# TaceoLabs/collaborative-circom

Measured on AMD Instinct MI355X. Metric: Groth16 constraints/sec (BN254, 2^22 R1CS), one REP3 party's prove, higher is better.
Workload: dtype u32; 1 GPU; synthetic R1CS 2^22 constraints-domain BN254, REP3 co-groth16 (configs[2]); num_constraints=4194302, domain_size=4194304, nnz=12582906, msm=8 G1 + 2 G2 of ~2^22 points, ntt=12

## Files before the change

collaborative-circom_amd/csrc/capi_internal.hpp:

```cpp
#pragma once
#include "common.hpp"
#include "curve.hpp"
#include "subgroup.hpp"
#include "host_ec64.hpp"
#include "ntt_kernels.hpp"
#include "plonk_kernels.hpp"

#include <cmath>
#include <chrono>
#include <map>
#include <set>
#include <mutex>
#include <vector>

using namespace cg;

namespace cg {
struct MsmSortPtrs { const uint32_t* sorted; const uint32_t* offsets; const uint32_t* counts; uint32_t cap; const uint32_t* overflow; };
template <class Fr> int msm_sort_launch(hipStream_t st, const Fr* d_scalars, size_t n, int c, int nwin, int shared, char* scratch, MsmSortPtrs* out, hipEvent_t* evs);
template <class Fr> int msm_sort_direct_launch(hipStream_t st, const Fr* d_scalars, size_t n, int c, int nwin, int shared, uint32_t cap, char* scratch, MsmSortPtrs* out, hipEvent_t* evs);
inline size_t msm_sort_direct_scratch_bytes(size_t n, int c, int nwin, int shared, uint32_t cap) {
    const size_t nbuckets = (size_t)(shared ? 1 : nwin) << (c - 1);
    return align_up(nbuckets * cap * 4) + 2 * align_up(nbuckets * 4) + align_up(((nbuckets + 2047) / 2048) * 4) + 256;
}
template <class F> int msm_accumulate_batch(hipStream_t st, const MsmAccSet* sets, int nsets, size_t n, int c, int nwin, bool shared, uint32_t cap, hipEvent_t* evs, uint32_t chunk_request, bool g2_slices);
template <class F> int msm_reduce_batch(hipStream_t st2, const MsmRedSet* sets, int nsets, size_t n, int c, int nwin, bool shared, uint32_t cap, hipEvent_t* ev_merged, int n_merged,
                                        hipEvent_t* evs, uint32_t chunk_request);
template <class F> size_t msm_acc_scratch_bytes(size_t n, int c, int nwin, bool shared, uint32_t chunk_request);
template <class F> int precompute_window_launch(hipStream_t st, const Affine<F>* d_src, Affine<F>* d_dst, size_t n, int c);
template <class F> int check_on_curve_launch(hipStream_t st, const Affine<F>* d_pts, size_t n, const F& b, unsigned long long* d_counters);
template <class F, class Fr> int check_subgroup_launch(hipStream_t st, const Affine<F>* d_pts, size_t n, unsigned long long* d_counters);
template <class F> int check_subgroup_fast_launch(hipStream_t st, const Affine<F>* d_pts, size_t n, const FastSubgroup<F>& c, unsigned long long* d_counters);
inline size_t msm_sort_scratch_bytes(size_t n, int c, int nwin) {
    const size_t nbuckets = (size_t)nwin << (c - 1);
    const size_t entries = (size_t)nwin * n;
    return 2 * align_up(entries * 4) + 3 * align_up(nbuckets * 4) + align_up(((nbuckets + 2047) / 2048) * 4) + align_up(entries * 8) + 2 * align_up(4096 * 4) + 256;
}
template <class F> int pack_bases_launch(hipStream_t st, const uint8_t* d_raw, size_t n, size_t stride, long inf_off, Affine<F>* d_dst);
template <class F> int gather_points_launch(hipStream_t st, Affine<F>* d_dst, const Affine<F>* d_src, const uint32_t* d_idx, size_t n);
template <class Fr> int launch_vec_gather_idx(hipStream_t st, Fr* out, const Fr* in, const uint32_t* idx, size_t n, uint32_t base);
template <class F> int synth_points_launch(hipStream_t st, const XYZZ<F>* d_lo, const XYZZ<F>* d_hi, int log_t, size_t n, Affine<F>* d_out);
template <class F, class Fr> int fixed_base_mul_launch(hipStream_t st, const Affine<F>& g, const Fr* d_scalars, size_t n, Affine<F>* d_tab, Affine<F>* d_out);
template <class Fr> int launch_vec_binary(hipStream_t st, int op, Fr* out, const Fr* a, const Fr* b, size_t n);
int chacha12_fr_rand_launch(hipStream_t st, const uint32_t* key8, const uint32_t* mod8, int modulus_bits, uint64_t word_pos, uint64_t n_pairs, uint64_t n,
                            void* d_cand, uint32_t* d_tiles, unsigned long long* d_result, void* d_out);
template <class Fr> int launch_rep3_mul_local(hipStream_t st, Fr* out, const Fr* aa, const Fr* ab, const Fr* ba, const Fr* bb, const Fr* mask, size_t n);
template <class Fr> int launch_distribute_powers(hipStream_t st, Fr* v, size_t n, const Fr* lo, const Fr* hi, int log_lo);
template <class Fr> int launch_vec_count_noncanonical(hipStream_t st, const Fr* v, size_t n, unsigned long long* n_bad);
template <class Fr> int launch_vec_fill(hipStream_t st, Fr* v, size_t n, const Fr& value);
template <class Fr> int launch_vec_affine(hipStream_t st, Fr* out, const Fr* a, size_t n, const Fr& c, const Fr& d);
template <class Fr> int launch_vec_gather_strided(hipStream_t st, Fr* out, const Fr* in, size_t n, size_t offset, size_t stride);
template <class Fr> int launch_vec_lincomb(hipStream_t st, Fr* out, long long out_off, long long out_stride, size_t n, const LincombArgs<Fr>& a);
template <class Fr> int launch_shamir_share(hipStream_t st, const Fr* secrets, const Fr* coeffs, long long coeff_off, long long coeff_stride, size_t n, int degree,
                                            const ShareOuts<Fr>& o, long long out_off, long long out_stride);
template <class Fr> int launch_plonk_r2_factors(hipStream_t st, const PlonkR2Args<Fr>& g, size_t n);
template <class Fr> int launch_prefix_scan(hipStream_t st, int op, Fr* out, const Fr* in, size_t n, Fr* scratch);
template <class Fr> int launch_vec_inverse(hipStream_t st, Fr* out, const Fr* in, size_t n);
template <class Fr> int launch_plonk_additions(hipStream_t st, const uint32_t* order, size_t n, const uint32_t* ids, const Fr* coeffs, const Fr* pub, uint32_t n_inputs, int pc,
                                               Fr* ext_a, Fr* ext_b, size_t n_priv);
// ... 220 lines not shown
```

collaborative-circom_amd/csrc/fr_impl.hpp:

```cpp
#pragma once
#include "common.hpp"
#include "ntt_kernels.hpp"
#include "vec_kernels.hpp"
#include "plonk_kernels.hpp"
#include "msm_sort_kernels.hpp"

namespace cg {

template <class Fr> int launch_vec_binary(hipStream_t st, int op, Fr* out, const Fr* a, const Fr* b, size_t n) {
    if (!n) return 0;
    if (op == 0) hipLaunchKernelGGL((k_vec_binary<Fr, 0>), dim3(grid_for(n)), dim3(256), 0, st, out, a, b, n);
    else if (op == 1) hipLaunchKernelGGL((k_vec_binary<Fr, 1>), dim3(grid_for(n)), dim3(256), 0, st, out, a, b, n);
    else hipLaunchKernelGGL((k_vec_binary<Fr, 2>), dim3(grid_for(n)), dim3(256), 0, st, out, a, b, n);
    HIPCHK(hipGetLastError());
    return 0;
}
template <class Fr> int launch_rep3_mul_local(hipStream_t st, Fr* out, const Fr* aa, const Fr* ab, const Fr* ba, const Fr* bb, const Fr* mask, size_t n) {
    if (!n) return 0;
    hipLaunchKernelGGL((k_rep3_mul_local<Fr>), dim3(grid_for(n)), dim3(256), 0, st, out, aa, ab, ba, bb, mask, n);
    HIPCHK(hipGetLastError());
    return 0;
}
template <class Fr> int launch_vec_count_noncanonical(hipStream_t st, const Fr* v, size_t n, unsigned long long* n_bad) {
    if (!n) return 0;
// ... 157 lines not shown
        hipLaunchKernelGGL((k_bitrev_finish_lazy_small<Fr>), dim3(grid_for(n), nvec), dim3(256), 0, st, dst, src, log_m, scale, c_lo, c_hi, log_lo);
    HIPCHK(hipGetLastError());
    return 0;
}
template <class Fr> int launch_bitrev_scale(hipStream_t st, NttVecs dst, NttVecs src, int nvec, size_t n, int log_m, const Fr* scale, const Fr* c_lo, const Fr* c_hi, int log_lo) {
    if (log_m >= 2 * BITREV_B)
        hipLaunchKernelGGL((k_bitrev_scale<Fr>), dim3((unsigned)(n >> (2 * BITREV_B)), nvec), dim3(256), 0, st, dst, src, log_m, scale, c_lo, c_hi, log_lo);
    else
        hipLaunchKernelGGL((k_bitrev_scale_small<Fr>), dim3(grid_for(n), nvec), dim3(256), 0, st, dst, src, log_m, scale, c_lo, c_hi, log_lo);
    HIPCHK(hipGetLastError());
    return 0;
}

struct MsmSortPtrs { const uint32_t* sorted; const uint32_t* offsets; const uint32_t* counts; uint32_t cap; const uint32_t* overflow; };
inline bool msm_sort_use_partition(size_t n, int c, int nwin, int shared) {
    const size_t nbuckets = (size_t)(shared ? 1 : nwin) << (c - 1);
    const size_t nregions = (nbuckets + ((size_t)1 << PART_REGION_LOG) - 1) >> PART_REGION_LOG;
    return (size_t)nwin * n >= ((size_t)1 << 21) && nregions >= 8 && nregions <= PART_MAX_REGIONS;
}
inline size_t msm_sort_scratch_bytes(size_t n, int c, int nwin) {
    const size_t nbuckets = (size_t)nwin << (c - 1);
    const size_t entries = (size_t)nwin * n, ntiles = (entries + PART_TILE - 1) / PART_TILE;
    return 2 * align_up(entries * 4) + 3 * align_up(nbuckets * 4) + align_up(((nbuckets + SCAN_TILE - 1) / SCAN_TILE) * 4) +
           align_up(entries * 8) + 2 * align_up(PART_MAX_REGIONS * 4) + 256;
}
template <class Fr> int msm_sort_launch(hipStream_t st, const Fr* d_scalars, size_t n, int c, int nwin, int shared, char* scratch, MsmSortPtrs* out, hipEvent_t* evs) {
    const size_t nbuckets = (size_t)(shared ? 1 : nwin) << (c - 1);
    size_t off = 0;
    auto take = [&](size_t bytes) { void* p = scratch + off; off += align_up(bytes); return p; };
    int32_t* digits = (int32_t*)take((size_t)nwin * n * 4);
    uint32_t* sorted = (uint32_t*)take((size_t)nwin * n * 4);
    uint32_t* counts = (uint32_t*)take(nbuckets * 4);
    uint32_t* cursors = (uint32_t*)take(nbuckets * 4);
    uint32_t* offsets = (uint32_t*)take(nbuckets * 4);
    const size_t ntiles = (nbuckets + SCAN_TILE - 1) / SCAN_TILE;
    uint32_t* tile_sums = (uint32_t*)take(ntiles * 4);
    if (evs) HIPCHK(hipEventRecord(evs[0], st));
    const bool no_small = !global_option(CG_GOPT_SORT_SMALL);
    static PerDeviceOnce attr_small; static std::atomic<bool> small_unavailable{false};
    if (shared && !no_small && !small_unavailable.load(std::memory_order_relaxed) && attr_small.pending()) {
        if (hipFuncSetAttribute((const void*)k_msm_sort_small<Fr>, hipFuncAttributeMaxDynamicSharedMemorySize, (int)((2 * SORT_SMALL_MAX_BUCKETS + 1024) * 4)) == hipSuccess) attr_small.mark();
        else { (void)hipGetLastError(); small_unavailable.store(true); }
    }
    if (shared && !no_small && !small_unavailable.load(std::memory_order_relaxed) && nbuckets <= SORT_SMALL_MAX_BUCKETS && (size_t)nwin * n <= SORT_SMALL_MAX_ENTRIES && n <= (1u << 24)) {
        const size_t lds = (2 * nbuckets + 1024) * 4;
        hipLaunchKernelGGL((k_msm_sort_small<Fr>), dim3(1), dim3(1024), lds, st, d_scalars, (uint32_t)n, c, nwin, counts, offsets, sorted);
        if (evs) HIPCHK(hipEventRecord(evs[1], st));
        HIPCHK(hipGetLastError());
        out->sorted = sorted; out->offsets = offsets; out->counts = counts; out->cap = 0; out->overflow = nullptr;
        return 0;
    }
    HIPCHK(hipMemsetAsync(counts, 0, align_up(nbuckets * 4) * 2, st));
    if (msm_sort_use_partition(n, c, nwin, shared)) {
        const size_t entries = (size_t)nwin * n, ptiles = (entries + PART_TILE - 1) / PART_TILE;
        const uint32_t nregions = (uint32_t)((nbuckets + ((size_t)1 << PART_REGION_LOG) - 1) >> PART_REGION_LOG);
        uint64_t* items = (uint64_t*)take(entries * 8);
        uint32_t* region_total = (uint32_t*)take(PART_MAX_REGIONS * 4);
        uint32_t* region_cursor = (uint32_t*)take(PART_MAX_REGIONS * 4);
        uint32_t* total_items = (uint32_t*)take(4);
        const unsigned itiles = (unsigned)(((entries + ITEM_TILE - 1) / ITEM_TILE + 7) / 8 * 8);
        HIPCHK(hipMemsetAsync(region_total, 0, nregions * 4, st));
        hipLaunchKernelGGL((k_msm_digits_only<Fr>), dim3(grid_for(n)), dim3(256), 0, st, d_scalars, n, c, nwin, digits);
        hipLaunchKernelGGL(k_part_hist, dim3((unsigned)ptiles), dim3(256), nregions * 4, st, digits, n, c, nwin, shared, nregions, region_total);
        hipLaunchKernelGGL(k_part_region_scan, dim3(1), dim3(1024), 0, st, region_total, nregions, region_cursor, total_items);
        const bool staged = global_option(CG_GOPT_SORT_STAGING) != 0;
        if (staged && nregions <= STAGE_MAX_REGIONS) {
            static PerDeviceOnce attr_set;
            if (attr_set.pending()) {
                HIPCHK(hipFuncSetAttribute((const void*)k_part_scatter_staged, hipFuncAttributeMaxDynamicSharedMemorySize, (int)part_staged_lds(STAGE_MAX_REGIONS)));
                HIPCHK(hipFuncSetAttribute((const void*)k_items_scatter_staged, hipFuncAttributeMaxDynamicSharedMemorySize, (int)ITEMS_STAGED_LDS));
                attr_set.mark();
            }
            hipLaunchKernelGGL(k_part_scatter_staged, dim3((unsigned)ptiles), dim3(STAGE_THREADS), part_staged_lds(nregions), st, digits, n, c, nwin, shared, nregions, region_cursor, items);
        } else
        hipLaunchKernelGGL(k_part_scatter, dim3((unsigned)ptiles), dim3(256), nregions * 4, st, digits, n, c, nwin, shared, nregions, region_cursor, items);
        hipLaunchKernelGGL(k_items_hist, dim3(itiles), dim3(256), 0, st, items, total_items, counts);
        hipLaunchKernelGGL(k_scan_tile_sums, dim3((unsigned)ntiles), dim3(256), 0, st, counts, tile_sums, nbuckets, 0xffffffffu);
        hipLaunchKernelGGL(k_scan_exclusive, dim3(1), dim3(1024), 0, st, tile_sums, tile_sums, ntiles);
        hipLaunchKernelGGL(k_scan_tiles, dim3((unsigned)ntiles), dim3(256), 0, st, counts, tile_sums, offsets, nbuckets, 0xffffffffu);
        if (staged && nregions <= STAGE_MAX_REGIONS) hipLaunchKernelGGL(k_items_scatter_staged, dim3(itiles), dim3(STAGE_THREADS), ITEMS_STAGED_LDS, st, items, total_items, offsets, cursors, sorted);
        else hipLaunchKernelGGL(k_items_scatter, dim3(itiles), dim3(256), 0, st, items, total_items, offsets, cursors, sorted);
        if (evs) HIPCHK(hipEventRecord(evs[1], st));
        HIPCHK(hipGetLastError());
        out->sorted = sorted; out->offsets = offsets; out->counts = counts; out->cap = 0; out->overflow = nullptr;
        return 0;
    }
    hipLaunchKernelGGL((k_msm_digits<Fr>), dim3(grid_for(n)), dim3(256), 0, st, d_scalars, n, c, nwin, shared, digits, counts);
    hipLaunchKernelGGL(k_scan_tile_sums, dim3((unsigned)ntiles), dim3(256), 0, st, counts, tile_sums, nbuckets, 0xffffffffu);
    hipLaunchKernelGGL(k_scan_exclusive, dim3(1), dim3(1024), 0, st, tile_sums, tile_sums, ntiles);
    hipLaunchKernelGGL(k_scan_tiles, dim3((unsigned)ntiles), dim3(256), 0, st, counts, tile_sums, offsets, nbuckets, 0xffffffffu);
    hipLaunchKernelGGL(k_msm_scatter, dim3(grid_for((size_t)nwin * n)), dim3(256), 0, st, digits, n, c, nwin, shared, offsets, cursors, sorted);
    if (evs) HIPCHK(hipEventRecord(evs[1], st));
    HIPCHK(hipGetLastError());
    out->sorted = sorted; out->offsets = offsets; out->counts = counts; out->cap = 0; out->overflow = nullptr;
    return 0;
}
inline size_t msm_sort_direct_scratch_bytes(size_t n, int c, int nwin, int shared, uint32_t cap) {
    const size_t nbuckets = (size_t)(shared ? 1 : nwin) << (c - 1);
    return align_up(nbuckets * cap * 4) + 2 * align_up(nbuckets * 4) + align_up(((nbuckets + SCAN_TILE - 1) / SCAN_TILE) * 4) + 256;
}
template <class Fr> int msm_sort_direct_launch(hipStream_t st, const Fr* d_scalars, size_t n, int c, int nwin, int shared, uint32_t cap, char* scratch, MsmSortPtrs* out, hipEvent_t* evs) {
    const size_t nbuckets = (size_t)(shared ? 1 : nwin) << (c - 1);
// ... 58 lines not shown
```

collaborative-circom_amd/csrc/msm_impl.hpp:

```cpp
#pragma once
#include <cstdlib>
#include "common.hpp"
#include "msm_kernels.hpp"

namespace cg {

template <class B> constexpr int bitsum_items() { return BITSUM_ITEMS; }
inline int bitsum_items_for(uint32_t nb) { return nb <= 1024u ? 1 : BITSUM_ITEMS; }
template <class B> uint32_t bitsum_groups(uint32_t nb) { const uint32_t it = (uint32_t)bitsum_items_for(nb); return std::max<uint32_t>(1, (nb / 2 + 256 * it - 1) / (256 * it)); }

template <class F> struct IsFp2 { static constexpr bool value = false; };
template <class B> struct IsFp2<Fp2<B>> { static constexpr bool value = true; };
template <class F> constexpr size_t acc_resident_lanes() { return IsFp2<F>::value ? 0 : (size_t)256 * (sizeof(F) == 32 ? 3 : 2) * 256; }

template <class F>
size_t msm_acc_scratch_bytes(size_t n, int c, int nwin, bool shared, uint32_t chunk_request) {
    typedef typename BucketOf<F>::type B;
    MsmGeom g = msm_geom(n, c, nwin, shared, acc_resident_lanes<F>(), chunk_request, IsFp2<F>::value);
    g.bit_groups = bitsum_groups<B>(g.nb);
    return align_up(g.nbuckets * sizeof(B)) + align_up((size_t)g.nchunks * sizeof(B)) + align_up((size_t)g.nchunks * 4) +
           align_up(std::max({(size_t)g.nsets * g.segs, (size_t)64 * g.bit_groups, g.grid_partials()}) * sizeof(B)) + align_up((size_t)std::max(g.ngroups, 64) * sizeof(XYZZ<F>));
}

template <class F>
// ... 9 lines not shown
        partials = (B*)take(std::max({(size_t)g.nsets * g.segs, (size_t)64 * g.bit_groups, g.grid_partials()}) * sizeof(B));
        wsums = (XYZZ<F>*)take((size_t)std::max(g.ngroups, 64) * sizeof(XYZZ<F>));
    }
};
template <class F>
MsmGeom msm_geom_of(size_t n, int c, int nwin, bool shared, uint32_t chunk_request) {
    MsmGeom g = msm_geom(n, c, nwin, shared, acc_resident_lanes<F>(), chunk_request, IsFp2<F>::value);
    g.bit_groups = bitsum_groups<typename BucketOf<F>::type>(g.nb);
    return g;
}

template <class F>
int msm_accumulate_batch(hipStream_t st, const MsmAccSet* sets, int nsets, size_t n, int c, int nwin, bool shared, uint32_t cap, hipEvent_t* evs, uint32_t chunk_request, bool g2_slices) {
    if (nsets < 1 || nsets > ACC_MAX_SETS) return fail(CG_ERR_ARG, "internal: accumulation batch size");
    const MsmGeom g = msm_geom_of<F>(n, c, nwin, shared, chunk_request);
    typedef typename BucketOf<F>::type B;
    AccSets<F> S{};
    for (int i = 0; i < nsets; i++) {
        const AccScratch<F> sc(sets[i].scratch, g);
        S.bases[i] = (const Affine<F>*)sets[i].bases; S.sorted[i] = sets[i].sorted; S.offsets[i] = sets[i].offsets; S.counts[i] = sets[i].counts;
        S.buckets[i] = sc.buckets; S.cont[i] = sc.cont; S.cont_bucket[i] = sc.cont_bucket;
        S.table_stride[i] = (uint32_t)sets[i].table_stride; S.may_have_inf[i] = sets[i].may_have_inf ? 1u : 0u;
    }
    const ptrdiff_t stride = nsets > 1 ? sets[1].scratch - sets[0].scratch : 0;
    bool one_fill = stride > 0 && (size_t)(nsets - 1) * (size_t)stride + g.nbuckets * sizeof(B) <= ((size_t)8 << 20);
    for (int i = 2; i < nsets && one_fill; i++) one_fill = sets[i].scratch - sets[i - 1].scratch == stride;
    if (one_fill) HIPCHK(hipMemsetAsync(S.buckets[0], 0, (size_t)(nsets - 1) * (size_t)stride + g.nbuckets * sizeof(B), st));
    else for (int i = 0; i < nsets; i++) HIPCHK(hipMemsetAsync(S.buckets[i], 0, g.nbuckets * sizeof(B), st));
    if (evs) HIPCHK(hipEventRecord(evs[0], st));
    auto launch_acc = [&](auto kern, int T, size_t lds) -> int {
        if (lds > 0) { if (int rc = ensure_dynamic_lds((const void*)kern, lds)) return rc; }
        for (int i = 0; i < nsets; i++)
            hipLaunchKernelGGL(kern, dim3((g.nchunks + T - 1) / T), dim3(T), lds, st, S.bases[i], S.sorted[i], S.offsets[i], S.counts[i],
                               (uint32_t)g.nbuckets, g.chunk_len, g.nchunks, S.table_stride[i], cap, S.buckets[i], S.cont[i], S.cont_bucket[i], S.may_have_inf[i]);
        return 0;
    };
    int rc_acc;
    const char* var_s = tune_env("CG_ACC_VARIANT");
    const int variant = var_s ? atoi(var_s) : 3;
    auto launch_pf = [&](auto kern, int T, size_t lds) -> int {
        if (lds > 0) { if (int rc = ensure_dynamic_lds((const void*)kern, lds)) return rc; }
        const uint32_t groups = (g.nchunks + T - 1) / T;
        const uint32_t slice = lds > 0 && g2_slices ? 256u * (uint32_t)std::max<size_t>(1, ((size_t)160 << 10) / lds) : groups;
        for (uint32_t first = 0; first < groups; first += slice)
            hipLaunchKernelGGL(kern, dim3(std::min(slice, groups - first), (unsigned)nsets), dim3(T), lds, st, S, (uint32_t)g.nbuckets, g.chunk_len, g.nchunks, first * (uint32_t)T);
        return 0;
    };
    constexpr bool g2 = IsFp2<F>::value;
    constexpr int MINW1 = sizeof(F) == 32 ? 3 : 2;
    const size_t lds2 = g2 ? (size_t)128 * 4 * sizeof(typename LazyOf<F>::type) : 0;
    if (variant && cap == 0) {
// ... 172 lines not shown
```

collaborative-circom_amd/csrc/msm_kernels.hpp:

```cpp
#pragma once
#include <type_traits>
#include "common.hpp"
#include "subgroup.hpp"
#include "curve.hpp"
#include "lazy29.hpp"
#include "vec_kernels.hpp"
#include "msm_sort_kernels.hpp"

namespace cg {

template <class A>
__device__ __forceinline__ A ld_struct(const A* p) {
    static_assert(sizeof(A) % 16 == 0, "");
    A r;
    const uint4* q = reinterpret_cast<const uint4*>(p);
    uint4* d = reinterpret_cast<uint4*>(&r);
    _Pragma("unroll") for (int i = 0; i < (int)(sizeof(A) / 16); i++) d[i] = q[i];
    return r;
}
template <class A>
__device__ __forceinline__ void st_struct(A* p, const A& r) {
    uint4* q = reinterpret_cast<uint4*>(p);
    const uint4* d = reinterpret_cast<const uint4*>(&r);
    _Pragma("unroll") for (int i = 0; i < (int)(sizeof(A) / 16); i++) q[i] = d[i];
// ... 466 lines not shown
        const bool neg = (e0 >> 31) != 0;
        pos++;
        if constexpr (PF != 3) { e0 = e1; e1 = e2; }
        if (may_have_inf && p.is_inf()) continue;
        acc_madd(acc, p.x, p.y, neg);
    }
    if (continuation) acc_store<F>(acc, cont + q); else acc_store<F>(acc, buckets + b);
}

constexpr uint32_t MERGE_DIRECT_MAX = 12;
template <class B>
struct RedSets {
    B* buckets[RED_MAX_SETS]; B* cont[RED_MAX_SETS]; uint32_t* cont_bucket[RED_MAX_SETS];
    const uint32_t* offsets[RED_MAX_SETS]; const uint32_t* counts[RED_MAX_SETS];
    B* partials[RED_MAX_SETS]; void* wsums[RED_MAX_SETS];
};
template <class B>
__global__ void __launch_bounds__(64) k_msm_merge_direct(const RedSets<B> S, uint32_t nbuckets, uint32_t chunk_len, uint32_t nchunks, uint32_t cap) {
    B* __restrict__ buckets = S.buckets[blockIdx.y]; const B* __restrict__ cont = S.cont[blockIdx.y]; uint32_t* __restrict__ cont_bucket = S.cont_bucket[blockIdx.y];
    const uint32_t* __restrict__ offsets = S.offsets[blockIdx.y]; const uint32_t* __restrict__ counts = S.counts[blockIdx.y];
    const uint32_t b = blockIdx.x * blockDim.x + threadIdx.x;
    if (b >= nbuckets) return;
    const uint32_t cnt = cap ? min(counts[b], cap) : counts[b];
    if (cnt == 0) return;
    const uint32_t first = offsets[b], last = first + cnt - 1;
    const uint32_t q0 = first / chunk_len + 1, q1 = last / chunk_len;
    if (q0 > q1 || q1 - q0 >= MERGE_DIRECT_MAX || q1 >= nchunks) return;
    B acc = ld_struct(buckets + b);
    for (uint32_t q = q0; q <= q1; q++) { acc = bk_add_inl(acc, ld_struct(cont + q)); cont_bucket[q] = 0xffffffffu; }
    st_struct(buckets + b, acc);
}
constexpr uint32_t MERGE_GROUP = 64;
template <class B>
__global__ void __launch_bounds__(64) k_msm_merge_cont_l1(const RedSets<B> S, uint32_t nchunks) {
    B* __restrict__ cont = S.cont[blockIdx.y]; const uint32_t* __restrict__ cont_bucket = S.cont_bucket[blockIdx.y];
    const uint32_t q = blockIdx.x * blockDim.x + threadIdx.x;
    if (q >= nchunks) return;
    const uint32_t b = cont_bucket[q];
    if (b == 0xffffffffu) return;
    const bool run_start = q == 0 || cont_bucket[q - 1] != b;
    if (!run_start && (q % MERGE_GROUP) != 0) return;
    const uint32_t next_head = (q / MERGE_GROUP + 1) * MERGE_GROUP;
    if (q + 1 >= nchunks || q + 1 >= next_head || cont_bucket[q + 1] != b) return;
    B acc = ld_struct(cont + q);
    for (uint32_t r = q + 1; r < nchunks && r < next_head && cont_bucket[r] == b; r++) acc = bk_add_inl(acc, ld_struct(cont + r));
    st_struct(cont + q, acc);
}
// ... 296 lines not shown
```

collaborative-circom_amd/csrc/msm_sort_kernels.hpp:

```cpp
#pragma once
#include "field.hpp"
#include "vec_kernels.hpp"

namespace cg {

template <class Fr>
__global__ void __launch_bounds__(256) k_msm_digits(const Fr* __restrict__ scalars, size_t n, int c, int nwin, int shared,
                                                    int32_t* __restrict__ digits, uint32_t* __restrict__ counts) {
    const uint32_t nb = 1u << (c - 1);
    const uint32_t mask = (1u << c) - 1;
    for (size_t i = (size_t)blockIdx.x * blockDim.x + threadIdx.x; i < n; i += (size_t)gridDim.x * blockDim.x) {
        Fr s = ld_fp(scalars + i).from_mont();
        uint32_t carry = 0;
        for (int w = 0; w < nwin; w++) {
            uint32_t d = (s.v[0] & mask) + carry;
            _Pragma("unroll") for (int l = 0; l < Fr::N; l++) {
                uint64_t two = ((uint64_t)(l + 1 < Fr::N ? s.v[l + 1] : 0u) << 32) | s.v[l];
                s.v[l] = (uint32_t)(two >> c);
            }
            int32_t dig;
            if (d > nb) { dig = (int32_t)d - (int32_t)(1u << c); carry = 1; } else { dig = (int32_t)d; carry = 0; }
            digits[(size_t)w * n + i] = dig;
            if (dig != 0) atomicAdd(&counts[(shared ? 0 : (size_t)w * nb) + (uint32_t)(dig < 0 ? -dig : dig) - 1], 1u);
        }
// ... 85 lines not shown
    for (uint32_t i = t; i < n; i += 1024) digits_of(i, [&](uint32_t, uint32_t b, bool) { atomicAdd(&cnt[b], 1u); });
    __syncthreads();
    const uint32_t chunk = (nb + 1023) / 1024, lo = min(t * chunk, nb), hi = min(lo + chunk, nb);
    uint32_t mine = 0;
    for (uint32_t b = lo; b < hi; b++) mine += cnt[b];
    part[t] = mine;
    __syncthreads();
    for (uint32_t off = 1; off < 1024; off <<= 1) {
        const uint32_t v = t >= off ? part[t - off] : 0;
        __syncthreads();
        part[t] += v;
        __syncthreads();
    }
    uint32_t run = part[t] - mine;
    for (uint32_t b = lo; b < hi; b++) { const uint32_t k = cnt[b]; offsets[b] = run; cur[b] = run; counts[b] = k; run += k; }
    __syncthreads();
    for (uint32_t i = t; i < n; i += 1024)
        digits_of(i, [&](uint32_t w, uint32_t b, bool neg) { sorted[atomicAdd(&cur[b], 1u)] = (w << 24) | i | (neg ? 0x80000000u : 0u); });
}

constexpr int PART_TILE = 16384;
constexpr int PART_REGION_LOG = 9;
constexpr int PART_MAX_REGIONS = 4096;

__device__ __forceinline__ bool part_decode(int32_t dig, size_t w, uint32_t i, uint32_t nb, int shared, uint32_t* bucket, uint32_t* payload) {
    if (dig == 0) return false;
    *bucket = (uint32_t)((shared ? 0 : w * nb) + (uint32_t)(dig < 0 ? -dig : dig) - 1);
    *payload = (shared ? ((uint32_t)w << 24) | i : i) | (dig < 0 ? 0x80000000u : 0u);
    return true;
}
template <class Fr>
__global__ void __launch_bounds__(256) k_msm_digits_only(const Fr* __restrict__ scalars, size_t n, int c, int nwin, int32_t* __restrict__ digits) {
    const uint32_t nb = 1u << (c - 1);
    const uint32_t mask = (1u << c) - 1;
    for (size_t i = (size_t)blockIdx.x * blockDim.x + threadIdx.x; i < n; i += (size_t)gridDim.x * blockDim.x) {
        Fr s = ld_fp(scalars + i).from_mont();
        uint32_t carry = 0;
        for (int w = 0; w < nwin; w++) {
            uint32_t d = (s.v[0] & mask) + carry;
            _Pragma("unroll") for (int l = 0; l < Fr::N; l++) {
                uint64_t two = ((uint64_t)(l + 1 < Fr::N ? s.v[l + 1] : 0u) << 32) | s.v[l];
                s.v[l] = (uint32_t)(two >> c);
            }
            int32_t dig;
            if (d > nb) { dig = (int32_t)d - (int32_t)(1u << c); carry = 1; } else { dig = (int32_t)d; carry = 0; }
            digits[(size_t)w * n + i] = dig;
        }
    }
}
static __global__ void __launch_bounds__(256) k_part_hist(const int32_t* __restrict__ digits, size_t n, int c, int nwin, int shared, uint32_t nregions,
                                                          uint32_t* __restrict__ region_total) {
    extern __shared__ uint32_t lds_cnt[];
    for (uint32_t r = threadIdx.x; r < nregions; r += 256) lds_cnt[r] = 0;
    __syncthreads();
    const uint32_t nb = 1u << (c - 1);
    const size_t total = (size_t)nwin * n, base = (size_t)blockIdx.x * PART_TILE;
    for (int k = 0; k < PART_TILE / 256; k++) {
        const size_t idx = base + (size_t)k * 256 + threadIdx.x;
        if (idx >= total) break;
        const size_t w = idx / n; uint32_t bucket, payload;
        if (part_decode(digits[idx], w, (uint32_t)(idx - w * n), nb, shared, &bucket, &payload)) atomicAdd(&lds_cnt[bucket >> PART_REGION_LOG], 1u);
    }
    __syncthreads();
    for (uint32_t r = threadIdx.x; r < nregions; r += 256) { const uint32_t v = lds_cnt[r]; if (v) atomicAdd(&region_total[r], v); }
}
static __global__ void __launch_bounds__(1024) k_part_region_scan(const uint32_t* __restrict__ region_total, uint32_t nregions, uint32_t* __restrict__ region_cursor,
                                                                  uint32_t* __restrict__ total_items) {
    __shared__ uint32_t part[1024];
    const uint32_t per = (nregions + 1023) / 1024;
    uint32_t v[4] = {0, 0, 0, 0}, mine = 0;
    for (uint32_t k = 0; k < per; k++) { const uint32_t r = threadIdx.x * per + k; if (r < nregions) { v[k] = region_total[r]; mine += v[k]; } }
    part[threadIdx.x] = mine;
    __syncthreads();
    for (int off = 1; off < 1024; off <<= 1) {
        uint32_t t = threadIdx.x >= (unsigned)off ? part[threadIdx.x - off] : 0;
        __syncthreads();
        part[threadIdx.x] += t;
        __syncthreads();
    }
    uint32_t run = threadIdx.x ? part[threadIdx.x - 1] : 0;
    if (threadIdx.x == 1023) *total_items = part[1023];
    for (uint32_t k = 0; k < per; k++) { const uint32_t r = threadIdx.x * per + k; if (r < nregions) { region_cursor[r] = run; run += v[k]; } }
}
static __global__ void __launch_bounds__(256) k_part_scatter(const int32_t* __restrict__ digits, size_t n, int c, int nwin, int shared, uint32_t nregions,
                                                             uint32_t* __restrict__ region_cursor, uint64_t* __restrict__ items) {
    extern __shared__ uint32_t lds_cnt[];
    for (uint32_t r = threadIdx.x; r < nregions; r += 256) lds_cnt[r] = 0;
    __syncthreads();
    const uint32_t nb = 1u << (c - 1);
    const size_t total = (size_t)nwin * n, base = (size_t)blockIdx.x * PART_TILE;
    for (int k = 0; k < PART_TILE / 256; k++) {
        const size_t idx = base + (size_t)k * 256 + threadIdx.x;
        if (idx >= total) break;
        const size_t w = idx / n; uint32_t bucket, payload;
        if (part_decode(digits[idx], w, (uint32_t)(idx - w * n), nb, shared, &bucket, &payload)) atomicAdd(&lds_cnt[bucket >> PART_REGION_LOG], 1u);
    }
    __syncthreads();
    for (uint32_t r = threadIdx.x; r < nregions; r += 256) { const uint32_t v = lds_cnt[r]; lds_cnt[r] = v ? atomicAdd(&region_cursor[r], v) : 0u; }
    __syncthreads();
    for (int k = 0; k < PART_TILE / 256; k++) {
        const size_t idx = base + (size_t)k * 256 + threadIdx.x;
        if (idx >= total) break;
        const size_t w = idx / n; uint32_t bucket, payload;
        if (part_decode(digits[idx], w, (uint32_t)(idx - w * n), nb, shared, &bucket, &payload)) {
            const uint32_t pos = atomicAdd(&lds_cnt[bucket >> PART_REGION_LOG], 1u);
            items[pos] = ((uint64_t)bucket << 32) | payload;
        }
    }
}
constexpr int ITEM_TILE = 16384;
constexpr uint32_t ITEM_WINDOW = 2048;
__device__ __forceinline__ uint32_t xcd_tile(uint32_t block, uint32_t nblocks) {
    const uint32_t per = (nblocks + 7) / 8;
    return (block & 7u) * per + (block >> 3);
}
static __global__ void __launch_bounds__(256) k_items_hist(const uint64_t* __restrict__ items, const uint32_t* __restrict__ total_items, uint32_t* __restrict__ counts) {
    __shared__ uint32_t cnt[ITEM_WINDOW];
    const size_t total = *total_items, base = (size_t)xcd_tile(blockIdx.x, gridDim.x) * ITEM_TILE;
    if (base >= total) return;
    for (uint32_t r = threadIdx.x; r < ITEM_WINDOW; r += 256) cnt[r] = 0;
    const uint32_t b0 = (uint32_t)(items[base] >> 32) & ~((1u << PART_REGION_LOG) - 1);
    __syncthreads();
    for (int k = 0; k < ITEM_TILE / 256; k++) {
        const size_t e = base + (size_t)k * 256 + threadIdx.x;
        if (e >= total) break;
        const uint32_t bucket = (uint32_t)(items[e] >> 32), d = bucket - b0;
        if (d < ITEM_WINDOW) atomicAdd(&cnt[d], 1u); else atomicAdd(&counts[bucket], 1u);
    }
    __syncthreads();
    for (uint32_t r = threadIdx.x; r < ITEM_WINDOW; r += 256) { const uint32_t v = cnt[r]; if (v) atomicAdd(&counts[b0 + r], v); }
// ... 5 lines not shown
    if (base >= total) return;
    for (uint32_t r = threadIdx.x; r < ITEM_WINDOW; r += 256) cnt[r] = 0;
    const uint32_t b0 = (uint32_t)(items[base] >> 32) & ~((1u << PART_REGION_LOG) - 1);
    __syncthreads();
    for (int k = 0; k < ITEM_TILE / 256; k++) {
        const size_t e = base + (size_t)k * 256 + threadIdx.x;
        if (e >= total) break;
        const uint32_t d = (uint32_t)(items[e] >> 32) - b0;
        if (d < ITEM_WINDOW) atomicAdd(&cnt[d], 1u);
    }
    __syncthreads();
    for (uint32_t r = threadIdx.x; r < ITEM_WINDOW; r += 256) { const uint32_t v = cnt[r]; cnt[r] = v ? offsets[b0 + r] + atomicAdd(&cursors[b0 + r], v) : 0u; }
    __syncthreads();
    for (int k = 0; k < ITEM_TILE / 256; k++) {
        const size_t e = base + (size_t)k * 256 + threadIdx.x;
        if (e >= total) break;
        const uint64_t it = items[e];
        const uint32_t bucket = (uint32_t)(it >> 32), d = bucket - b0;
        const uint32_t pos = d < ITEM_WINDOW ? atomicAdd(&cnt[d], 1u) : offsets[bucket] + atomicAdd(&cursors[bucket], 1u);
        sorted[pos] = (uint32_t)it;
    }
}

constexpr int STAGE_THREADS = 1024;
constexpr int STAGE_PER_LANE = PART_TILE / STAGE_THREADS;
constexpr uint32_t STAGE_MAX_REGIONS = 2048;
inline size_t part_staged_lds(uint32_t nregions) { return (size_t)(2 * nregions + 32) * 4 + (size_t)PART_TILE * 8; }
constexpr size_t ITEMS_STAGED_LDS = (size_t)(2 * ITEM_WINDOW + 32) * 4 + (size_t)ITEM_TILE * 6;
__device__ __forceinline__ uint32_t stage_block_scan(uint32_t v, uint32_t* scratch, uint32_t* total) {
    const int lane = threadIdx.x & 63, wave = threadIdx.x >> 6;
    uint32_t inc = v;
    _Pragma("unroll") for (int off = 1; off < 64; off <<= 1) { const uint32_t t = __shfl_up(inc, off, 64); if (lane >= off) inc += t; }
    if (lane == 63) scratch[wave] = inc;
    __syncthreads();
    if (wave == 0) {
        uint32_t w = lane < STAGE_THREADS / 64 ? scratch[lane] : 0, winc = w;
        _Pragma("unroll") for (int off = 1; off < STAGE_THREADS / 64; off <<= 1) { const uint32_t t = __shfl_up(winc, off, 64); if (lane >= off) winc += t; }
        if (lane < STAGE_THREADS / 64) scratch[lane] = winc - w;
        if (lane == STAGE_THREADS / 64 - 1) scratch[STAGE_THREADS / 64] = winc;
    }
    __syncthreads();
    const uint32_t r = scratch[wave] + inc - v;
    *total = scratch[STAGE_THREADS / 64];
    __syncthreads();
    return r;
}
static __global__ void __launch_bounds__(STAGE_THREADS) k_part_scatter_staged(const int32_t* __restrict__ digits, size_t n, int c, int nwin, int shared, uint32_t nregions,
                                                                            uint32_t* __restrict__ region_cursor, uint64_t* __restrict__ items) {
    extern __shared__ uint32_t lds_u32[];
    uint32_t* cnt = lds_u32;
    uint32_t* delta = cnt + nregions;
    uint32_t* scratch = delta + nregions;
    uint64_t* stage = reinterpret_cast<uint64_t*>(scratch + 32);
    for (uint32_t r = threadIdx.x; r < nregions; r += STAGE_THREADS) cnt[r] = 0;
    const uint32_t nb = 1u << (c - 1);
    const size_t total = (size_t)nwin * n, base = (size_t)blockIdx.x * PART_TILE;
    int32_t dig[STAGE_PER_LANE];
    _Pragma("unroll") for (int k = 0; k < STAGE_PER_LANE; k++) {
        const size_t idx = base + (size_t)k * STAGE_THREADS + threadIdx.x;
        dig[k] = idx < total ? digits[idx] : 0;
    }
    __syncthreads();
    uint32_t bucket[STAGE_PER_LANE], payload[STAGE_PER_LANE], rank[STAGE_PER_LANE];
    _Pragma("unroll") for (int k = 0; k < STAGE_PER_LANE; k++) {
        const size_t idx = base + (size_t)k * STAGE_THREADS + threadIdx.x;
        const size_t w = idx / n;
        bucket[k] = 0xffffffffu; payload[k] = 0; rank[k] = 0;
        if (part_decode(dig[k], w, (uint32_t)(idx - w * n), nb, shared, &bucket[k], &payload[k])) rank[k] = atomicAdd(&cnt[bucket[k] >> PART_REGION_LOG], 1u);
        else bucket[k] = 0xffffffffu;
    }
    __syncthreads();
    const uint32_t per = (nregions + STAGE_THREADS - 1) / STAGE_THREADS;
    uint32_t v[2] = {0, 0}, mine = 0;
    for (uint32_t j = 0; j < per; j++) { const uint32_t r = threadIdx.x * per + j; if (r < nregions) { v[j] = cnt[r]; mine += v[j]; } }
    uint32_t tile_items;
    uint32_t run = stage_block_scan(mine, scratch, &tile_items);
    for (uint32_t j = 0; j < per; j++) {
        const uint32_t r = threadIdx.x * per + j;
        if (r < nregions) { cnt[r] = run; delta[r] = (v[j] ? atomicAdd(&region_cursor[r], v[j]) : 0u) - run; run += v[j]; }
    }
    __syncthreads();
    _Pragma("unroll") for (int k = 0; k < STAGE_PER_LANE; k++)
        if (bucket[k] != 0xffffffffu) stage[cnt[bucket[k] >> PART_REGION_LOG] + rank[k]] = ((uint64_t)bucket[k] << 32) | payload[k];
    __syncthreads();
    for (uint32_t s = threadIdx.x; s < tile_items; s += STAGE_THREADS) {
        const uint64_t it = stage[s];
        items[delta[(uint32_t)(it >> 32) >> PART_REGION_LOG] + s] = it;
    }
}
static __global__ void __launch_bounds__(STAGE_THREADS) k_items_scatter_staged(const uint64_t* __restrict__ items, const uint32_t* __restrict__ total_items,
                                                                             const uint32_t* __restrict__ offsets, uint32_t* __restrict__ cursors, uint32_t* __restrict__ sorted) {
    extern __shared__ uint32_t lds_u32[];
    uint32_t* cnt = lds_u32;
    uint32_t* delta = cnt + ITEM_WINDOW;
    uint32_t* scratch = delta + ITEM_WINDOW;
    uint32_t* stage = scratch + 32;
    uint16_t* slot = reinterpret_cast<uint16_t*>(stage + ITEM_TILE);
    const size_t total = *total_items, base = (size_t)xcd_tile(blockIdx.x, gridDim.x) * ITEM_TILE;
    if (base >= total) return;
    for (uint32_t r = threadIdx.x; r < ITEM_WINDOW; r += STAGE_THREADS) cnt[r] = 0;
    uint64_t it[STAGE_PER_LANE];
    _Pragma("unroll") for (int k = 0; k < STAGE_PER_LANE; k++) {
        const size_t e = base + (size_t)k * STAGE_THREADS + threadIdx.x;
        it[k] = e < total ? items[e] : ~(uint64_t)0;
    }
    const uint32_t b0 = (uint32_t)(items[base] >> 32) & ~((1u << PART_REGION_LOG) - 1);
    __syncthreads();
    uint32_t rank[STAGE_PER_LANE];
    _Pragma("unroll") for (int k = 0; k < STAGE_PER_LANE; k++) {
        rank[k] = 0;
// ... 54 lines not shown
```

Measured before the change: 61.37 million constraints/s.

## Fuse scalar digit recoding into partition sort and drop bucket memsets

The MSM partition sort no longer materialises a digits array. The histogram and scatter kernels now load each scalar, convert it from Montgomery form and recode its signed windows inline, tiling by scalars instead of by (window, scalar) entries. The three-kernel bucket offset scan is replaced by a per-region offsets kernel seeded from region bases. The bucket buffer memsets are removed, and the merge kernel instead writes infinity into empty buckets. Together these are meant to cut global traffic and launch count, at the cost of recomputing the recode twice per scalar and relying on the merge kernel to initialise every bucket.

Result: no change. 61.96 million constraints/s (median of 6 runs) (+0.9%).

```diff
diff --git a/collaborative-circom_amd/csrc/capi_internal.hpp b/collaborative-circom_amd/csrc/capi_internal.hpp
--- a/collaborative-circom_amd/csrc/capi_internal.hpp
+++ b/collaborative-circom_amd/csrc/capi_internal.hpp
@@ -34,7 +34,7 @@
 inline size_t msm_sort_scratch_bytes(size_t n, int c, int nwin) {
     const size_t nbuckets = (size_t)nwin << (c - 1);
     const size_t entries = (size_t)nwin * n;
-    return 2 * align_up(entries * 4) + 3 * align_up(nbuckets * 4) + align_up(((nbuckets + 2047) / 2048) * 4) + align_up(entries * 8) + 2 * align_up(4096 * 4) + 256;
+    return 2 * align_up(entries * 4) + 3 * align_up(nbuckets * 4) + align_up(((nbuckets + 2047) / 2048) * 4) + align_up(entries * 8) + 3 * align_up(4096 * 4) + 256;
 }
 template <class F> int pack_bases_launch(hipStream_t st, const uint8_t* d_raw, size_t n, size_t stride, long inf_off, Affine<F>* d_dst);
 template <class F> int gather_points_launch(hipStream_t st, Affine<F>* d_dst, const Affine<F>* d_src, const uint32_t* d_idx, size_t n);
diff --git a/collaborative-circom_amd/csrc/fr_impl.hpp b/collaborative-circom_amd/csrc/fr_impl.hpp
--- a/collaborative-circom_amd/csrc/fr_impl.hpp
+++ b/collaborative-circom_amd/csrc/fr_impl.hpp
@@ -203,7 +203,7 @@
     const size_t nbuckets = (size_t)nwin << (c - 1);
     const size_t entries = (size_t)nwin * n, ntiles = (entries + PART_TILE - 1) / PART_TILE;
     return 2 * align_up(entries * 4) + 3 * align_up(nbuckets * 4) + align_up(((nbuckets + SCAN_TILE - 1) / SCAN_TILE) * 4) +
-           align_up(entries * 8) + 2 * align_up(PART_MAX_REGIONS * 4) + 256;
+           align_up(entries * 8) + 3 * align_up(PART_MAX_REGIONS * 4) + 256;
 }
 template <class Fr> int msm_sort_launch(hipStream_t st, const Fr* d_scalars, size_t n, int c, int nwin, int shared, char* scratch, MsmSortPtrs* out, hipEvent_t* evs) {
     const size_t nbuckets = (size_t)(shared ? 1 : nwin) << (c - 1);
@@ -233,32 +233,32 @@
     }
     HIPCHK(hipMemsetAsync(counts, 0, align_up(nbuckets * 4) * 2, st));
     if (msm_sort_use_partition(n, c, nwin, shared)) {
-        const size_t entries = (size_t)nwin * n, ptiles = (entries + PART_TILE - 1) / PART_TILE;
+        const size_t entries = (size_t)nwin * n;
+        const uint32_t tile_scalars = part_tile_scalars(nwin);
+        const size_t ptiles = (n + tile_scalars - 1) / tile_scalars;
         const uint32_t nregions = (uint32_t)((nbuckets + ((size_t)1 << PART_REGION_LOG) - 1) >> PART_REGION_LOG);
         uint64_t* items = (uint64_t*)take(entries * 8);
         uint32_t* region_total = (uint32_t*)take(PART_MAX_REGIONS * 4);
         uint32_t* region_cursor = (uint32_t*)take(PART_MAX_REGIONS * 4);
+        uint32_t* region_base = (uint32_t*)take(PART_MAX_REGIONS * 4);
         uint32_t* total_items = (uint32_t*)take(4);
         const unsigned itiles = (unsigned)(((entries + ITEM_TILE - 1) / ITEM_TILE + 7) / 8 * 8);
         HIPCHK(hipMemsetAsync(region_total, 0, nregions * 4, st));
-        hipLaunchKernelGGL((k_msm_digits_only<Fr>), dim3(grid_for(n)), dim3(256), 0, st, d_scalars, n, c, nwin, digits);
-        hipLaunchKernelGGL(k_part_hist, dim3((unsigned)ptiles), dim3(256), nregions * 4, st, digits, n, c, nwin, shared, nregions, region_total);
-        hipLaunchKernelGGL(k_part_region_scan, dim3(1), dim3(1024), 0, st, region_total, nregions, region_cursor, total_items);
+        hipLaunchKernelGGL((k_part_hist<Fr>), dim3((unsigned)ptiles), dim3(256), nregions * 4, st, d_scalars, n, c, nwin, shared, nregions, tile_scalars, region_total);
+        hipLaunchKernelGGL(k_part_region_scan, dim3(1), dim3(1024), 0, st, region_total, nregions, region_cursor, region_base, total_items);
         const bool staged = global_option(CG_GOPT_SORT_STAGING) != 0;
         if (staged && nregions <= STAGE_MAX_REGIONS) {
             static PerDeviceOnce attr_set;
             if (attr_set.pending()) {
-                HIPCHK(hipFuncSetAttribute((const void*)k_part_scatter_staged, hipFuncAttributeMaxDynamicSharedMemorySize, (int)part_staged_lds(STAGE_MAX_REGIONS)));
+                HIPCHK(hipFuncSetAttribute((const void*)k_part_scatter_staged<Fr>, hipFuncAttributeMaxDynamicSharedMemorySize, (int)part_staged_lds(STAGE_MAX_REGIONS)));
                 HIPCHK(hipFuncSetAttribute((const void*)k_items_scatter_staged, hipFuncAttributeMaxDynamicSharedMemorySize, (int)ITEMS_STAGED_LDS));
                 attr_set.mark();
             }
-            hipLaunchKernelGGL(k_part_scatter_staged, dim3((unsigned)ptiles), dim3(STAGE_THREADS), part_staged_lds(nregions), st, digits, n, c, nwin, shared, nregions, region_cursor, items);
+            hipLaunchKernelGGL((k_part_scatter_staged<Fr>), dim3((unsigned)ptiles), dim3(STAGE_THREADS), part_staged_lds(nregions), st, d_scalars, n, c, nwin, shared, nregions, tile_scalars, region_cursor, items);
         } else
-        hipLaunchKernelGGL(k_part_scatter, dim3((unsigned)ptiles), dim3(256), nregions * 4, st, digits, n, c, nwin, shared, nregions, region_cursor, items);
+        hipLaunchKernelGGL((k_part_scatter<Fr>), dim3((unsigned)ptiles), dim3(256), nregions * 4, st, d_scalars, n, c, nwin, shared, nregions, tile_scalars, region_cursor, items);
         hipLaunchKernelGGL(k_items_hist, dim3(itiles), dim3(256), 0, st, items, total_items, counts);
-        hipLaunchKernelGGL(k_scan_tile_sums, dim3((unsigned)ntiles), dim3(256), 0, st, counts, tile_sums, nbuckets, 0xffffffffu);
-        hipLaunchKernelGGL(k_scan_exclusive, dim3(1), dim3(1024), 0, st, tile_sums, tile_sums, ntiles);
-        hipLaunchKernelGGL(k_scan_tiles, dim3((unsigned)ntiles), dim3(256), 0, st, counts, tile_sums, offsets, nbuckets, 0xffffffffu);
+        hipLaunchKernelGGL(k_part_region_offsets, dim3(nregions), dim3(1 << PART_REGION_LOG), 0, st, counts, region_base, (uint32_t)nbuckets, offsets);
         if (staged && nregions <= STAGE_MAX_REGIONS) hipLaunchKernelGGL(k_items_scatter_staged, dim3(itiles), dim3(STAGE_THREADS), ITEMS_STAGED_LDS, st, items, total_items, offsets, cursors, sorted);
         else hipLaunchKernelGGL(k_items_scatter, dim3(itiles), dim3(256), 0, st, items, total_items, offsets, cursors, sorted);
         if (evs) HIPCHK(hipEventRecord(evs[1], st));
diff --git a/collaborative-circom_amd/csrc/msm_impl.hpp b/collaborative-circom_amd/csrc/msm_impl.hpp
--- a/collaborative-circom_amd/csrc/msm_impl.hpp
+++ b/collaborative-circom_amd/csrc/msm_impl.hpp
@@ -55,11 +55,6 @@
         S.buckets[i] = sc.buckets; S.cont[i] = sc.cont; S.cont_bucket[i] = sc.cont_bucket;
         S.table_stride[i] = (uint32_t)sets[i].table_stride; S.may_have_inf[i] = sets[i].may_have_inf ? 1u : 0u;
     }
-    const ptrdiff_t stride = nsets > 1 ? sets[1].scratch - sets[0].scratch : 0;
-    bool one_fill = stride > 0 && (size_t)(nsets - 1) * (size_t)stride + g.nbuckets * sizeof(B) <= ((size_t)8 << 20);
-    for (int i = 2; i < nsets && one_fill; i++) one_fill = sets[i].scratch - sets[i - 1].scratch == stride;
-    if (one_fill) HIPCHK(hipMemsetAsync(S.buckets[0], 0, (size_t)(nsets - 1) * (size_t)stride + g.nbuckets * sizeof(B), st));
-    else for (int i = 0; i < nsets; i++) HIPCHK(hipMemsetAsync(S.buckets[i], 0, g.nbuckets * sizeof(B), st));
     if (evs) HIPCHK(hipEventRecord(evs[0], st));
     auto launch_acc = [&](auto kern, int T, size_t lds) -> int {
         if (lds > 0) { if (int rc = ensure_dynamic_lds((const void*)kern, lds)) return rc; }
diff --git a/collaborative-circom_amd/csrc/msm_kernels.hpp b/collaborative-circom_amd/csrc/msm_kernels.hpp
--- a/collaborative-circom_amd/csrc/msm_kernels.hpp
+++ b/collaborative-circom_amd/csrc/msm_kernels.hpp
@@ -512,7 +512,7 @@
     const uint32_t b = blockIdx.x * blockDim.x + threadIdx.x;
     if (b >= nbuckets) return;
     const uint32_t cnt = cap ? min(counts[b], cap) : counts[b];
-    if (cnt == 0) return;
+    if (cnt == 0) { st_struct(buckets + b, bk_inf<B>()); return; }
     const uint32_t first = offsets[b], last = first + cnt - 1;
     const uint32_t q0 = first / chunk_len + 1, q1 = last / chunk_len;
     if (q0 > q1 || q1 - q0 >= MERGE_DIRECT_MAX || q1 >= nchunks) return;
diff --git a/collaborative-circom_amd/csrc/msm_sort_kernels.hpp b/collaborative-circom_amd/csrc/msm_sort_kernels.hpp
--- a/collaborative-circom_amd/csrc/msm_sort_kernels.hpp
+++ b/collaborative-circom_amd/csrc/msm_sort_kernels.hpp
@@ -131,6 +131,8 @@
 constexpr int PART_TILE = 16384;
 constexpr int PART_REGION_LOG = 9;
 constexpr int PART_MAX_REGIONS = 4096;
+constexpr int STAGE_THREADS = 1024;
+inline uint32_t part_tile_scalars(int nwin) { return (uint32_t)(PART_TILE / nwin < STAGE_THREADS ? PART_TILE / nwin : STAGE_THREADS); }
 
 __device__ __forceinline__ bool part_decode(int32_t dig, size_t w, uint32_t i, uint32_t nb, int shared, uint32_t* bucket, uint32_t* payload) {
     if (dig == 0) return false;
@@ -157,24 +159,38 @@
         }
     }
 }
-static __global__ void __launch_bounds__(256) k_part_hist(const int32_t* __restrict__ digits, size_t n, int c, int nwin, int shared, uint32_t nregions,
-                                                          uint32_t* __restrict__ region_total) {
+template <class Fr, class Fn>
+__device__ __forceinline__ void part_recode(Fr s, uint32_t i, int c, int nwin, int shared, Fn&& f) {
+    const uint32_t nb = 1u << (c - 1), mask = (1u << c) - 1;
+    uint32_t carry = 0;
+    for (int w = 0; w < nwin; w++) {
+        const uint32_t d = (s.v[0] & mask) + carry;
+        _Pragma("unroll") for (int l = 0; l < Fr::N; l++) {
+            const uint64_t two = ((uint64_t)(l + 1 < Fr::N ? s.v[l + 1] : 0u) << 32) | s.v[l];
+            s.v[l] = (uint32_t)(two >> c);
+        }
+        carry = d > nb ? 1u : 0u;
+        uint32_t bucket, payload;
+        if (part_decode(carry ? (int32_t)d - (int32_t)(1u << c) : (int32_t)d, (size_t)w, i, nb, shared, &bucket, &payload)) f(bucket, payload);
+    }
+}
+template <class Fr>
+__global__ void __launch_bounds__(256) k_part_hist(const Fr* __restrict__ scalars, size_t n, int c, int nwin, int shared, uint32_t nregions, uint32_t tile_scalars,
+                                                   uint32_t* __restrict__ region_total) {
     extern __shared__ uint32_t lds_cnt[];
     for (uint32_t r = threadIdx.x; r < nregions; r += 256) lds_cnt[r] = 0;
     __syncthreads();
-    const uint32_t nb = 1u << (c - 1);
-    const size_t total = (size_t)nwin * n, base = (size_t)blockIdx.x * PART_TILE;
-    for (int k = 0; k < PART_TILE / 256; k++) {
-        const size_t idx = base + (size_t)k * 256 + threadIdx.x;
-        if (idx >= total) break;
-        const size_t w = idx / n; uint32_t bucket, payload;
-        if (part_decode(digits[idx], w, (uint32_t)(idx - w * n), nb, shared, &bucket, &payload)) atomicAdd(&lds_cnt[bucket >> PART_REGION_LOG], 1u);
+    const size_t base = (size_t)blockIdx.x * tile_scalars;
+    for (uint32_t k = threadIdx.x; k < tile_scalars; k += 256) {
+        const size_t i = base + k;
+        if (i >= n) break;
+        part_recode(ld_fp(scalars + i).from_mont(), (uint32_t)i, c, nwin, shared, [&](uint32_t bucket, uint32_t) { atomicAdd(&lds_cnt[bucket >> PART_REGION_LOG], 1u); });
     }
     __syncthreads();
     for (uint32_t r = threadIdx.x; r < nregions; r += 256) { const uint32_t v = lds_cnt[r]; if (v) atomicAdd(&region_total[r], v); }
 }
 static __global__ void __launch_bounds__(1024) k_part_region_scan(const uint32_t* __restrict__ region_total, uint32_t nregions, uint32_t* __restrict__ region_cursor,
-                                                                  uint32_t* __restrict__ total_items) {
+                                                                  uint32_t* __restrict__ region_base, uint32_t* __restrict__ total_items) {
     __shared__ uint32_t part[1024];
     const uint32_t per = (nregions + 1023) / 1024;
     uint32_t v[4] = {0, 0, 0, 0}, mine = 0;
@@ -189,32 +205,42 @@
     }
     uint32_t run = threadIdx.x ? part[threadIdx.x - 1] : 0;
     if (threadIdx.x == 1023) *total_items = part[1023];
-    for (uint32_t k = 0; k < per; k++) { const uint32_t r = threadIdx.x * per + k; if (r < nregions) { region_cursor[r] = run; run += v[k]; } }
-}
-static __global__ void __launch_bounds__(256) k_part_scatter(const int32_t* __restrict__ digits, size_t n, int c, int nwin, int shared, uint32_t nregions,
-                                                             uint32_t* __restrict__ region_cursor, uint64_t* __restrict__ items) {
+    for (uint32_t k = 0; k < per; k++) { const uint32_t r = threadIdx.x * per + k; if (r < nregions) { region_cursor[r] = run; region_base[r] = run; run += v[k]; } }
+}
+static __global__ void __launch_bounds__(1 << PART_REGION_LOG) k_part_region_offsets(const uint32_t* __restrict__ counts, const uint32_t* __restrict__ region_base,
+                                                                                    uint32_t nbuckets, uint32_t* __restrict__ offsets) {
+    __shared__ uint32_t wave_sum[(1 << PART_REGION_LOG) / 64];
+    const uint32_t b = (blockIdx.x << PART_REGION_LOG) + threadIdx.x, lane = threadIdx.x & 63u, wave = threadIdx.x >> 6;
+    const uint32_t v = b < nbuckets ? counts[b] : 0u;
+    uint32_t inc = v;
+    _Pragma("unroll") for (int off = 1; off < 64; off <<= 1) { const uint32_t t = __shfl_up(inc, off, 64); if ((int)lane >= off) inc += t; }
+    if (lane == 63u) wave_sum[wave] = inc;
+    __syncthreads();
+    uint32_t run = region_base[blockIdx.x];
+    for (uint32_t k = 0; k < wave; k++) run += wave_sum[k];
+    if (b < nbuckets) offsets[b] = run + inc - v;
+}
+template <class Fr>
+__global__ void __launch_bounds__(256) k_part_scatter(const Fr* __restrict__ scalars, size_t n, int c, int nwin, int shared, uint32_t nregions, uint32_t tile_scalars,
+                                                      uint32_t* __restrict__ region_cursor, uint64_t* __restrict__ items) {
     extern __shared__ uint32_t lds_cnt[];
     for (uint32_t r = threadIdx.x; r < nregions; r += 256) lds_cnt[r] = 0;
     __syncthreads();
-    const uint32_t nb = 1u << (c - 1);
-    const size_t total = (size_t)nwin * n, base = (size_t)blockIdx.x * PART_TILE;
-    for (int k = 0; k < PART_TILE / 256; k++) {
-        const size_t idx = base + (size_t)k * 256 + threadIdx.x;
-        if (idx >= total) break;
-        const size_t w = idx / n; uint32_t bucket, payload;
-        if (part_decode(digits[idx], w, (uint32_t)(idx - w * n), nb, shared, &bucket, &payload)) atomicAdd(&lds_cnt[bucket >> PART_REGION_LOG], 1u);
+    const size_t base = (size_t)blockIdx.x * tile_scalars;
+    for (uint32_t k = threadIdx.x; k < tile_scalars; k += 256) {
+        const size_t i = base + k;
+        if (i >= n) break;
+        part_recode(ld_fp(scalars + i).from_mont(), (uint32_t)i, c, nwin, shared, [&](uint32_t bucket, uint32_t) { atomicAdd(&lds_cnt[bucket >> PART_REGION_LOG], 1u); });
     }
     __syncthreads();
     for (uint32_t r = threadIdx.x; r < nregions; r += 256) { const uint32_t v = lds_cnt[r]; lds_cnt[r] = v ? atomicAdd(&region_cursor[r], v) : 0u; }
     __syncthreads();
-    for (int k = 0; k < PART_TILE / 256; k++) {
-        const size_t idx = base + (size_t)k * 256 + threadIdx.x;
-        if (idx >= total) break;
-        const size_t w = idx / n; uint32_t bucket, payload;
-        if (part_decode(digits[idx], w, (uint32_t)(idx - w * n), nb, shared, &bucket, &payload)) {
-            const uint32_t pos = atomicAdd(&lds_cnt[bucket >> PART_REGION_LOG], 1u);
-            items[pos] = ((uint64_t)bucket << 32) | payload;
-        }
+    for (uint32_t k = threadIdx.x; k < tile_scalars; k += 256) {
+        const size_t i = base + k;
+        if (i >= n) break;
+        part_recode(ld_fp(scalars + i).from_mont(), (uint32_t)i, c, nwin, shared, [&](uint32_t bucket, uint32_t payload) {
+            items[atomicAdd(&lds_cnt[bucket >> PART_REGION_LOG], 1u)] = ((uint64_t)bucket << 32) | payload;
+        });
     }
 }
 constexpr int ITEM_TILE = 16384;
@@ -266,7 +292,6 @@
     }
 }
 
-constexpr int STAGE_THREADS = 1024;
 constexpr int STAGE_PER_LANE = PART_TILE / STAGE_THREADS;
 constexpr uint32_t STAGE_MAX_REGIONS = 2048;
 inline size_t part_staged_lds(uint32_t nregions) { return (size_t)(2 * nregions + 32) * 4 + (size_t)PART_TILE * 8; }
@@ -289,30 +314,21 @@
     __syncthreads();
     return r;
 }
-static __global__ void __launch_bounds__(STAGE_THREADS) k_part_scatter_staged(const int32_t* __restrict__ digits, size_t n, int c, int nwin, int shared, uint32_t nregions,
-                                                                            uint32_t* __restrict__ region_cursor, uint64_t* __restrict__ items) {
+template <class Fr>
+__global__ void __launch_bounds__(STAGE_THREADS) k_part_scatter_staged(const Fr* __restrict__ scalars, size_t n, int c, int nwin, int shared, uint32_t nregions, uint32_t tile_scalars,
+                                                                     uint32_t* __restrict__ region_cursor, uint64_t* __restrict__ items) {
     extern __shared__ uint32_t lds_u32[];
     uint32_t* cnt = lds_u32;
     uint32_t* delta = cnt + nregions;
     uint32_t* scratch = delta + nregions;
     uint64_t* stage = reinterpret_cast<uint64_t*>(scratch + 32);
     for (uint32_t r = threadIdx.x; r < nregions; r += STAGE_THREADS) cnt[r] = 0;
-    const uint32_t nb = 1u << (c - 1);
-    const size_t total = (size_t)nwin * n, base = (size_t)blockIdx.x * PART_TILE;
-    int32_t dig[STAGE_PER_LANE];
-    _Pragma("unroll") for (int k = 0; k < STAGE_PER_LANE; k++) {
-        const size_t idx = base + (size_t)k * STAGE_THREADS + threadIdx.x;
-        dig[k] = idx < total ? digits[idx] : 0;
-    }
-    __syncthreads();
-    uint32_t bucket[STAGE_PER_LANE], payload[STAGE_PER_LANE], rank[STAGE_PER_LANE];
-    _Pragma("unroll") for (int k = 0; k < STAGE_PER_LANE; k++) {
-        const size_t idx = base + (size_t)k * STAGE_THREADS + threadIdx.x;
-        const size_t w = idx / n;
-        bucket[k] = 0xffffffffu; payload[k] = 0; rank[k] = 0;
-        if (part_decode(dig[k], w, (uint32_t)(idx - w * n), nb, shared, &bucket[k], &payload[k])) rank[k] = atomicAdd(&cnt[bucket[k] >> PART_REGION_LOG], 1u);
-        else bucket[k] = 0xffffffffu;
-    }
+    const size_t i = (size_t)blockIdx.x * tile_scalars + threadIdx.x;
+    const bool live = threadIdx.x < tile_scalars && i < n;
+    Fr s = Fr::zero();
+    if (live) s = ld_fp(scalars + i).from_mont();
+    __syncthreads();
+    if (live) part_recode(s, (uint32_t)i, c, nwin, shared, [&](uint32_t bucket, uint32_t) { atomicAdd(&cnt[bucket >> PART_REGION_LOG], 1u); });
     __syncthreads();
     const uint32_t per = (nregions + STAGE_THREADS - 1) / STAGE_THREADS;
     uint32_t v[2] = {0, 0}, mine = 0;
@@ -324,12 +340,13 @@
         if (r < nregions) { cnt[r] = run; delta[r] = (v[j] ? atomicAdd(&region_cursor[r], v[j]) : 0u) - run; run += v[j]; }
     }
     __syncthreads();
-    _Pragma("unroll") for (int k = 0; k < STAGE_PER_LANE; k++)
-        if (bucket[k] != 0xffffffffu) stage[cnt[bucket[k] >> PART_REGION_LOG] + rank[k]] = ((uint64_t)bucket[k] << 32) | payload[k];
-    __syncthreads();
-    for (uint32_t s = threadIdx.x; s < tile_items; s += STAGE_THREADS) {
-        const uint64_t it = stage[s];
-        items[delta[(uint32_t)(it >> 32) >> PART_REGION_LOG] + s] = it;
+    if (live) part_recode(s, (uint32_t)i, c, nwin, shared, [&](uint32_t bucket, uint32_t payload) {
+        stage[atomicAdd(&cnt[bucket >> PART_REGION_LOG], 1u)] = ((uint64_t)bucket << 32) | payload;
+    });
+    __syncthreads();
+    for (uint32_t t = threadIdx.x; t < tile_items; t += STAGE_THREADS) {
+        const uint64_t it = stage[t];
+        items[delta[(uint32_t)(it >> 32) >> PART_REGION_LOG] + t] = it;
     }
 }
 static __global__ void __launch_bounds__(STAGE_THREADS) k_items_scatter_staged(const uint64_t* __restrict__ items, const uint32_t* __restrict__ total_items,
```
